# juhyeonkim95/Mitsuba3DopplerToF

Hardware: AMD Instinct MI355X
Metric: Mpaths/s (whole node), Doppler Cornell 512x512 64spp (higher is better)
Workload: dtype f32

## Files before the change

include/dtof.h:

```cpp
#ifndef DTOF_H
#define DTOF_H
#include <stdint.h>
#include <stddef.h>

#ifdef __cplusplus
extern "C" {
#endif

#define DTOF_OK            0
#define DTOF_ERR_INVALID   1
#define DTOF_ERR_HIP       2
#define DTOF_ERR_CANCELLED 3

typedef struct dtof_scene   dtof_scene;
typedef struct dtof_sampler dtof_sampler;

const char *dtof_version(void);
const char *dtof_last_error(void);

int dtof_scene_load_file(const char *path, const char *const *param_names, const char *const *param_values,
                         int n_params, dtof_scene **out);
int dtof_scene_load_string(const char *xml, const char *const *param_names, const char *const *param_values,
                           int n_params, dtof_scene **out);
void dtof_scene_destroy(dtof_scene *scene);
// ... 146 lines not shown
void dtof_sampler_destroy(dtof_sampler *s);
int  dtof_sampler_seed(dtof_sampler *s, uint32_t seed, uint32_t wavefront_size);
int  dtof_sampler_set_samples_per_wavefront(dtof_sampler *s, uint32_t spw);
int  dtof_sampler_advance(dtof_sampler *s);
int  dtof_sampler_next_1d(dtof_sampler *s, float *out);
int  dtof_sampler_next_2d(dtof_sampler *s, float *out_xy);
int  dtof_sampler_next_1d_correlate(dtof_sampler *s, const uint8_t *correlate, int correlate_all, float *out);
int  dtof_sampler_next_2d_correlate(dtof_sampler *s, const uint8_t *correlate, int correlate_all, float *out_xy);
int  dtof_sampler_next_1d_time(dtof_sampler *s, int strategy, float antithetic_shift, int stratify_each_interval, float *out);
int  dtof_sampler_get_state(dtof_sampler *s, uint32_t *out7);
int  dtof_sampler_fork(const dtof_sampler *s, dtof_sampler **out);
int  dtof_sampler_clone(const dtof_sampler *s, dtof_sampler **out);
int  dtof_sampler_set_sample_count(dtof_sampler *s, uint32_t sample_count);
int  dtof_sampler_seeded(const dtof_sampler *s);
uint32_t dtof_sampler_wavefront_size(const dtof_sampler *s);
uint32_t dtof_sampler_sample_count(const dtof_sampler *s);

int dtof_eval_modulation(dtof_scene *scene, int mode, const float *t, const float *len, float *out, uint32_t n);

int dtof_ray_intersect(dtof_scene *scene, uint32_t n, const float *rays8, float *out19, int32_t *ids3);
int dtof_ray_intersect_uv(dtof_scene *scene, uint32_t n, const float *rays8, float *out19, int32_t *ids3, float *uv4);
int dtof_ray_test(dtof_scene *scene, uint32_t n, const float *rays8, int32_t *occluded);
int dtof_flat_query(dtof_scene *scene, int form, int any, uint32_t n, const float *rays8, float *out3, int32_t *ids);

#define DTOF_COMP_MICROFACET_EVAL          0
#define DTOF_COMP_MICROFACET_PDF           1
#define DTOF_COMP_MICROFACET_G1            2
#define DTOF_COMP_MICROFACET_SAMPLE        3
#define DTOF_COMP_FRESNEL                  4
#define DTOF_COMP_FRESNEL_CONDUCTOR        5
#define DTOF_COMP_RFILTER                  6
#define DTOF_COMP_WARP_COSINE_HEMISPHERE   7
#define DTOF_COMP_WARP_DISK_CONCENTRIC     8
#define DTOF_COMP_WARP_UNIFORM_TRIANGLE    9
#define DTOF_COMP_WARP_UNIFORM_SPHERE     10
#define DTOF_COMP_COORDINATE_SYSTEM       11
#define DTOF_COMP_TEA_FLOAT32             12
#define DTOF_COMP_MATH                    13
int dtof_eval_component(int component, const float *params, int n_params, const float *in, int in_stride, float *out, int out_stride, uint32_t n);

#ifdef __cplusplus
}
#endif
#endif
```

mitsuba3dopplertof_amd/__init__.py:

```python
import ctypes as C
import os

import numpy as np

__all__ = ["load_file", "load_string", "load_dict", "Scene", "Integrator", "Sampler", "DtofError", "render",
           "render_multi_pass", "to_tof_image", "lib_path", "ETimeSampling", "velocity_map_variants", "MOMENT_PLANES", "aov_channels", "AOV_TYPES"]

_HERE = os.path.dirname(os.path.abspath(__file__))
_LIB = None


class DtofError(RuntimeError):
    pass


class ETimeSampling:
    UNIFORM, STRATIFIED, ANTITHETIC, ANTITHETIC_MIRROR, PERIODIC, REGULAR = 0, 1, 2, 3, 4, 5


class _Stats(C.Structure):
    _fields_ = [("n_paths", C.c_uint64), ("n_bounces", C.c_uint64), ("n_shadow_rays", C.c_uint64),
                ("ms_total", C.c_double), ("ms_generate", C.c_double), ("ms_trace", C.c_double),
                ("ms_shade", C.c_double), ("ms_shadow", C.c_double), ("ms_splat", C.c_double),
                ("n_launches_trace", C.c_uint32), ("n_launches_shade", C.c_uint32), ("n_launches_shadow", C.c_uint32),
# ... 96 lines not shown
    L.dtof_sampler_seeded.argtypes = [vp]
    L.dtof_eval_modulation.argtypes = [vp, C.c_int, vp, vp, vp, C.c_uint32]
    L.dtof_eval_component.argtypes = [C.c_int, vp, C.c_int, vp, C.c_int, vp, C.c_int, C.c_uint32]
    L.dtof_render_rows_async.argtypes = [vp, C.c_uint32, C.c_uint32, C.c_int32, C.c_int32, vp, C.c_int, vp]
    L.dtof_clear_async.argtypes = [vp, vp, C.c_size_t]
    L.dtof_camera_rays.argtypes = [vp, C.c_uint32, vp, vp]
    L.dtof_bsdf_eval.argtypes = [vp, C.c_uint32, C.c_uint32, vp, vp]
    L.dtof_bsdf_eval_ex.argtypes = [vp, C.c_uint32, C.c_int, C.c_uint32, vp, vp]
    L.dtof_scene_set_stream.argtypes = [vp, vp]
    L.dtof_scene_set_film_layout.argtypes = [vp, C.c_int32, C.c_uint64]
    L.dtof_render_stripes_async.argtypes = [vp, C.c_uint32, C.c_uint32, C.c_int32, C.c_int32, C.c_int32, vp, C.c_int, vp]
    L.dtof_develop_async.argtypes = [vp, vp, vp, C.c_int64]
    L.dtof_async_collect.argtypes = [vp, vp, vp, C.c_uint32, vp]
    L.dtof_ray_intersect.argtypes = [vp, C.c_uint32, vp, vp, vp]
    L.dtof_ray_intersect_uv.argtypes = [vp, C.c_uint32, vp, vp, vp, vp]
    L.dtof_ray_test.argtypes = [vp, C.c_uint32, vp, vp]
    rows, stripes = [vp, C.c_uint32, C.c_uint32, C.c_int32, C.c_int32, vp, C.c_int, vp], [vp, C.c_uint32, C.c_uint32, C.c_int32, C.c_int32, C.c_int32, vp, C.c_int, vp]
    for name, args in (("dtof_render_variants", [vp, C.c_uint32, C.c_uint32, vp, C.c_int, vp, C.POINTER(_Stats)]),
                       ("dtof_render_rows_variants", rows + [C.POINTER(_Stats)]), ("dtof_render_rows_variants_async", rows),
                       ("dtof_render_stripes_variants", stripes + [C.POINTER(_Stats)]), ("dtof_render_stripes_variants_async", stripes),
                       ("dtof_sample_lanes_variants", [vp, C.c_uint32, C.c_uint32, vp, C.c_int, C.c_uint64, C.c_uint64, vp, vp, vp]),
                       ("dtof_emitter_eval", [vp, C.c_int, C.c_int, C.c_int32, C.c_uint32, vp, vp]),
                       ("dtof_flat_query", [vp, C.c_int, C.c_int, C.c_uint32, vp, vp, vp]),
                       ("dtof_develop_accumulate_async", [vp, vp, C.c_int32, C.c_uint64, vp, C.c_int64, C.c_int]),
                       ("dtof_velocity_map_async", [vp, vp, C.c_int, vp, vp, C.c_uint32, C.c_double, C.c_double, C.c_int64, vp, vp, vp]),
                       ("dtof_velocity_map_variants", [vp, C.c_int, vp]),
                       ("dtof_render_velocity_map", [vp, C.c_uint32, C.c_uint32, vp, C.c_int, C.c_double, C.c_double, vp, vp, vp, C.POINTER(_Stats)]),
                       ("dtof_render_velocity_map_f64", [vp, C.c_uint32, C.c_uint32, vp, C.c_int, C.c_double, C.c_double, vp, vp, vp, C.POINTER(_Stats)]),
                       ("dtof_render_variants_f64", [vp, C.c_uint32, C.c_uint32, vp, C.c_int, vp, vp, C.POINTER(_Stats)]),
                       ("dtof_render_rows_variants_f64", rows[:-1] + [vp, C.c_int32, C.c_uint64, C.POINTER(_Stats)]),
                       ("dtof_develop_f64_async", [vp, vp, vp, C.c_int64]), ("dtof_develop_rgba_f64_async", [vp, vp, vp, vp, C.c_int64]),
                       ("dtof_moment_planes", [C.c_int]),
                       ("dtof_render_moments", [vp, C.c_uint32, C.c_uint32, C.c_uint32, vp, C.c_int, C.c_int, vp, C.POINTER(_Stats)]),
                       ("dtof_aov_parse", [C.c_char_p, vp, C.c_int, C.POINTER(C.c_int), vp, C.c_size_t, C.POINTER(C.c_int)]),
                       ("dtof_scene_get_aovs", [vp, vp, C.c_size_t]),
                       ("dtof_render_aovs", [vp, C.c_uint32, C.c_uint32, C.c_uint32, vp, C.c_int, C.c_int, vp, C.POINTER(_Stats)]),
                       ("dtof_sample_aov_lanes", [vp, C.c_uint32, C.c_uint32, vp, C.c_int, C.c_uint64, C.c_uint64, vp, vp])):
        if hasattr(L, name):
            getattr(L, name).argtypes = args
    _LIB = L
    return L


FLAT_GEOMETRY = np.array([[1, 0, 0,  0, 1, 0,  0, 0, 1,  1, 0, 0,  0, 1, 0,  0, 0, 1]], np.float32)


# ... 437 lines not shown

    def ray_intersect(self, o, d, time=0.0, maxt=None):
        rays = self._rays(o, d, time, maxt)
        out, ids, uv = np.zeros((len(rays), 19), np.float32), np.zeros((len(rays), 3), np.int32), np.zeros((len(rays), 4), np.float32)
        _check(_lib().dtof_ray_intersect_uv(self._h, len(rays), rays.ctypes.data, out.ctypes.data, ids.ctypes.data, uv.ctypes.data))
        return {"t": out[:, 0], "p": out[:, 1:4], "n": out[:, 4:7], "sh_n": out[:, 7:10], "sh_s": out[:, 10:13], "sh_t": out[:, 13:16],
                "wi": out[:, 16:19], "ids": ids, "uv": uv[:, 0:2], "prim_uv": uv[:, 2:4], "prim_index": ids[:, 2], "valid": ids[:, 0] >= 0}

    def ray_test(self, o, d, time=0.0, maxt=None):
        rays = self._rays(o, d, time, maxt)
        occ = np.zeros(len(rays), np.int32)
        _check(_lib().dtof_ray_test(self._h, len(rays), rays.ctypes.data, occ.ctypes.data))
        return occ != 0

    FLAT_FORMS = {"generic": 0, "one_wall": 1, "shape": 2}

    def flat_query(self, rays8, form=0, any=False):
        rays = np.ascontiguousarray(rays8, np.float32).reshape(-1, 8)
        form = self.FLAT_FORMS.get(form, form)
        out, ids = np.zeros((len(rays), 3), np.float32), np.zeros(len(rays), np.int32)
        _check(_lib().dtof_flat_query(self._h, int(form), 1 if any else 0, len(rays), rays.ctypes.data, None if any else out.ctypes.data, ids.ctypes.data))
        return ids if any else {"t": out[:, 0], "u": out[:, 1], "v": out[:, 2], "obj": ids}

    def cancel(self):
        _lib().dtof_cancel(self._h)


COMPONENTS = {"microfacet_eval": (0, 1), "microfacet_pdf": (1, 1), "microfacet_g1": (2, 1), "microfacet_sample": (3, 4), "fresnel": (4, 4),
              "fresnel_conductor": (5, 1), "rfilter": (6, 1), "warp_cosine_hemisphere": (7, 3), "warp_disk_concentric": (8, 2),
              "warp_uniform_triangle": (9, 2), "warp_uniform_sphere": (10, 3), "coordinate_system": (11, 6), "tea_float32": (12, 1), "math": (13, 1)}


def eval_component(name, inputs, params=()):
    comp, n_out = COMPONENTS[name]
    x = np.ascontiguousarray(np.atleast_2d(np.asarray(inputs, np.float32)))
    p = np.ascontiguousarray(np.asarray(params, np.float32).reshape(-1))
    out = np.zeros((len(x), n_out), np.float32)
    _check(_lib().dtof_eval_component(comp, p.ctypes.data if p.size else None, p.size, x.ctypes.data, x.shape[1], out.ctypes.data, n_out, len(x)))
    return out


class Integrator:

    def __init__(self, props):
        self.props = dict(props)
        self._h = C.c_void_p()
# ... 174 lines not shown
```

mitsuba3dopplertof_amd/csrc/dtof_flat_query.h:

```cpp
#pragma once
#include "dtof_kernels.h"

namespace dtof {

constexpr uint32_t kFlatQueryForms = 3;
constexpr uint32_t flat_query_facts(int form) { return form == 2 ? kHeadlineShapeFacts & kFactsFlatTable : form == 1 ? (uint32_t) kFactOneWall : 0u; }
void launch_flat_query(const uint8_t *scene, uint32_t scene_bytes, uint32_t flat_off, uint32_t flat_objects, uint32_t memo_obj, int form, bool any,
                       const float *rays, float *out3, int32_t *ids, uint32_t n, hipStream_t s);

}
```

mitsuba3dopplertof_amd/csrc/dtof_flat_query.hip:

```cpp
#include "dtof_device.h"
#include "dtof_flat_query.h"

namespace dtof {

static_assert(kHeadlineShapeFacts == 0 || (flat_query_facts(2) & kFactFlatShape) != 0, "form 2 is the shaped walk");

template <bool ANY, uint32_t FACTS>
__global__ __launch_bounds__(kShadeBlock) void k_flat_query(const uint8_t *scene, uint32_t scene_bytes, uint32_t stage_words, uint32_t flat_off, uint32_t flat_objects,
                                                             uint32_t memo_obj, const float *rays, float *out3, int32_t *ids, uint32_t n) {
    extern __shared__ uint4 lds[];
    constexpr bool F_ONE_WALL = (FACTS & kFactOneWall) != 0;
    const uint8_t *base = stage_scene(scene, scene_bytes, lds);
    SceneView sv = make_view(base);
    const bool have_memo = F_ONE_WALL || memo_obj != 0xffffffffu;
    sv.memo_obj = memo_obj; sv.memo = (float *) (lds + stage_words) + threadIdx.x; sv.memo_m = have_memo;
    const uint32_t i = blockIdx.x * kShadeBlock + threadIdx.x;
    if (i >= n) return;
    const float *r = rays + (size_t) i * 8;
    const V3 o = mk(r[0], r[1], r[2]), d = mk(r[3], r[4], r[5]);
    const float time = r[6], maxt = r[7];
    float memo_m[12], memo_inv[12];
    if (have_memo) instance_memo_fill(sv, time, memo_m, memo_inv);
    Hit h;
    const bool found = trace_flat<ANY, true, FACTS>(sv, (ConstBytes) scene + flat_off, flat_off, flat_objects, nullptr, o, d, time, maxt, h);
    if (ANY) { ids[i] = found ? 1 : 0; return; }
    float *w = out3 + (size_t) i * 3;
    ids[i] = found ? (int32_t) h.obj : -1;
    w[0] = found ? h.t : u2f(0x7f800000u); w[1] = found ? h.u : 0.f; w[2] = found ? h.v : 0.f;
}

template <uint32_t FACTS>
static void launch_form(bool any, uint32_t grid, uint32_t lds, hipStream_t s, const uint8_t *scene, uint32_t scene_bytes, uint32_t stage_words, uint32_t flat_off,
                        uint32_t flat_objects, uint32_t memo_obj, const float *rays, float *out3, int32_t *ids, uint32_t n) {
    if (any) hipLaunchKernelGGL((k_flat_query<true, FACTS>), dim3(grid), dim3(kShadeBlock), lds, s, scene, scene_bytes, stage_words, flat_off, flat_objects, memo_obj, rays, out3, ids, n);
    else hipLaunchKernelGGL((k_flat_query<false, FACTS>), dim3(grid), dim3(kShadeBlock), lds, s, scene, scene_bytes, stage_words, flat_off, flat_objects, memo_obj, rays, out3, ids, n);
}

void launch_flat_query(const uint8_t *scene, uint32_t scene_bytes, uint32_t flat_off, uint32_t flat_objects, uint32_t memo_obj, int form, bool any,
                       const float *rays, float *out3, int32_t *ids, uint32_t n, hipStream_t s) {
    if (!n) return;
    const uint32_t stage_words = (scene_bytes + 15u) / 16u;
    const uint32_t lds = ShadeLds::classic(stage_words, true, memo_obj != 0xffffffffu, 1u).without_stack();
    if (scene_bytes > 16u * 1024u) throw std::runtime_error("dtof_flat_query: the scene does not fit the LDS stage");
    const uint32_t grid = (n + kShadeBlock - 1u) / kShadeBlock;
    if (form == 2) launch_form<flat_query_facts(2)>(any, grid, lds, s, scene, scene_bytes, stage_words, flat_off, flat_objects, memo_obj, rays, out3, ids, n);
    else if (form == 1) launch_form<flat_query_facts(1)>(any, grid, lds, s, scene, scene_bytes, stage_words, flat_off, flat_objects, memo_obj, rays, out3, ids, n);
    else launch_form<flat_query_facts(0)>(any, grid, lds, s, scene, scene_bytes, stage_words, flat_off, flat_objects, memo_obj, rays, out3, ids, n);
}

}
```

mitsuba3dopplertof_amd/csrc/dtof_kernels.h:

```cpp
#pragma once
#include <stdint.h>
#include <hip/hip_runtime.h>
#include "dtof_math.h"

namespace dtof {

constexpr uint32_t kChunkBlocks = 8;
constexpr uint32_t kMaxInline = 4;
constexpr int kMaxOffsets = 4;

struct RenderParams {
    float s2c[16];
    float cam_to_world[12];
    float near_clip, far_clip, shutter_open, shutter_open_time;
    int32_t orthographic;
    float aperture_radius, focus_distance;
    int32_t crop_x, crop_y, crop_w, crop_h;
    float scale_x, scale_y, offset_x, offset_y;
    int32_t filter; float filter_radius, inv_radius;
    float gauss_coeff[10];
    float filter_b, filter_c;
    uint32_t base_seed, seed, seed_value;
    uint32_t spp, spp_log2;
    uint32_t tcn, pcn;
// ... 146 lines not shown
#ifndef DTOF_HEADLINE_C2
#define DTOF_HEADLINE_C2 0x3e000
#endif
constexpr uint32_t kHeadlineC2Facts = (DTOF_HEADLINE_C2) != 0 && kHeadlineFusedFacts != 0 ? (kHeadlineFusedFacts | (DTOF_HEADLINE_C2)) : 0u;
static_assert(((DTOF_HEADLINE_C2) & ~kFactsSampling) == 0, "DTOF_HEADLINE_C2 names route facts only (bits 13 and up)");
#ifndef DTOF_HEADLINE_SHAPE_COUNT
#define DTOF_HEADLINE_SHAPE_COUNT 5
#endif
#ifndef DTOF_HEADLINE_SHAPE_WALL
#define DTOF_HEADLINE_SHAPE_WALL 2
#endif
constexpr uint32_t kHeadlineShapeFacts = (DTOF_HEADLINE_SHAPE_COUNT) != 0 && (kHeadlineC2Facts & kFactOneWall) != 0 ? (kHeadlineC2Facts | flat_shape_fact(DTOF_HEADLINE_SHAPE_COUNT, DTOF_HEADLINE_SHAPE_WALL)) : 0u;
static_assert((DTOF_HEADLINE_SHAPE_COUNT) == 0 || (kHeadlineC2Facts & kFactOneWall) == 0 || (kHeadlineShapeFacts & kFactFlatShape) != 0, "a shape has 1 .. 8 objects and the wall among them");
#ifndef DTOF_HEADLINE_PAIR
#define DTOF_HEADLINE_PAIR 1
#endif
#ifndef DTOF_STREAM_JUMPS
#define DTOF_STREAM_JUMPS 1
#endif
#ifndef DTOF_PAIR_SAMPLES
#define DTOF_PAIR_SAMPLES 1
#endif
constexpr uint32_t kHeadlinePairFacts = DTOF_HEADLINE_PAIR && kHeadlineShapeFacts != 0 ? (kHeadlineShapeFacts | kFactPairSamples) : 0u;
#ifndef DTOF_FLAT_SHAPE_ANY
#define DTOF_FLAT_SHAPE_ANY 1
#endif
#ifndef DTOF_FLAT_SHAPE_CLOSEST
#define DTOF_FLAT_SHAPE_CLOSEST 1
#endif
#ifndef DTOF_WALL_FRAMES
#define DTOF_WALL_FRAMES 1
#endif
#ifndef DTOF_RESIDENT_FACTS
#define DTOF_RESIDENT_FACTS 0x37f
#endif
constexpr uint32_t kResidentFacts = DTOF_RESIDENT_FACTS;

struct ShadeLaunch { bool staged; int mode; uint32_t waves, grid, lds, lds_flat; hipStream_t stream; ShadeArgs args; uint32_t facts; };
uint32_t launch_shade_plain(bool area, bool k4, const ShadeLaunch &L);
void launch_shade_mesh(bool area, bool k4, const ShadeLaunch &L);
void launch_shade_spec1(bool k4, const ShadeLaunch &L);
void launch_shade_spec2(bool k4, const ShadeLaunch &L);
uint32_t launch_shade_resident0(bool area, bool k4, const ShadeLaunch &L);
void launch_shade_resident1(bool k4, const ShadeLaunch &L);
void launch_shade_resident2(bool k4, const ShadeLaunch &L);

// ... 70 lines not shown
```

mitsuba3dopplertof_amd/csrc/dtof_render.hip:

```cpp
#include "../../include/dtof.h"
#include "dtof_kernels.h"
#include "dtof_reconstruct.h"
#include "dtof_film64.h"
#include "dtof_moments.h"
#include "dtof_aov.h"
#include "dtof_flat_query.h"
#include "dtof_scene.h"
#include "dtof_math.h"
#include <atomic>
#include <dlfcn.h>
#include <cstdio>
#include <cstring>
#include <cstdlib>
#include <cmath>
#include <string>
#include <memory>
#include <vector>

using namespace dtof;

namespace {

thread_local std::string g_last_error;

// ... 1778 lines not shown
int dtof_flat_query(dtof_scene *sc, int form, int any, uint32_t n, const float *rays8, float *out3, int32_t *ids) {
    return guarded([&] {
        if (!sc || (n && (!rays8 || !ids || (!any && !out3)))) throw std::runtime_error("null argument");
        if (form < 0 || form >= (int) kFlatQueryForms) throw std::runtime_error("dtof_flat_query: form must be 0 (generic), 1 (one_wall) or 2 (shape)");
        if (n > (1u << 24)) throw std::runtime_error("dtof_flat_query: more than 2^24 rays in one call");
        const SceneTraits t = scene_traits(*sc);
        const FlatChoice c = flat_choice(t, t.blas_triangles <= 32768 && sc->host.textures.empty(), true, true);
        if (c.flat_objects == 0) throw std::runtime_error("dtof_flat_query: the scene has no flat table (rectangles only, at most 8 objects, fused pipeline)");
        if (form >= 1 && !(c.facts & kFactOneWall)) throw std::runtime_error("dtof_flat_query: the one_wall and shape forms need exactly one instance that holds one rectangle");
        if (form == 2 && (flat_query_facts(2) == 0 || (c.facts & kFlatShapeFields) != (flat_query_facts(2) & kFlatShapeFields)))
            throw std::runtime_error("dtof_flat_query: the shape form is compiled for a table of " + std::to_string(flat_shape_count(flat_query_facts(2))) + " rectangles with the wall at index " +
                                     std::to_string(flat_shape_wall(flat_query_facts(2))) + ", this table has " + std::to_string(c.flat_objects) + " and " + std::to_string(c.memo_obj));
        ensure_device(sc);
        DevBuf<float> dr, dout; DevBuf<int32_t> dids;
        dr.ensure((size_t) n * 8); dout.ensure(any ? 1 : (size_t) n * 3); dids.ensure(n);
        if (n) HIP_CHECK(hipMemcpy(dr.p, rays8, (size_t) n * 32, hipMemcpyHostToDevice));
        launch_flat_query(sc->d_blob.p, (uint32_t) sc->blob.size(), t.flat_off, c.flat_objects, c.memo_obj, form, any != 0, dr.p, dout.p, dids.p, n, nullptr);
        HIP_CHECK(hipGetLastError());
        if (n && !any) HIP_CHECK(hipMemcpy(out3, dout.p, (size_t) n * 12, hipMemcpyDeviceToHost));
        if (n) HIP_CHECK(hipMemcpy(ids, dids.p, (size_t) n * 4, hipMemcpyDeviceToHost));
    });
}

#ifdef DTOF_TRAVERSAL_STATS
int dtof_debug_traversal_stats_n(unsigned long long *out8, uint32_t n) {
    return guarded([&] {
        HIP_CHECK(hipDeviceSynchronize());
        unsigned long long all[kTravStats];
        if (!read_traversal_stats(all)) throw HipError("hipMemcpyFromSymbol(g_trav_stats) failed");
        for (uint32_t i = 0; i < n && i < kTravStats; ++i) out8[i] = all[i];
    });
}
int dtof_debug_traversal_stats(unsigned long long *out8) { return dtof_debug_traversal_stats_n(out8, 16); }
#endif

}
```

mitsuba3dopplertof_amd/csrc/dtof_shade.h:

```cpp
#pragma once
#include "dtof_device.h"
#include <atomic>
#include <initializer_list>
#include <type_traits>

namespace dtof {


DTOF_D uint32_t wave_append(bool pred, uint32_t &running) {
    const uint64_t mask = __ballot(pred);
    const uint32_t slot = running + (uint32_t) __popcll(mask & ((1ull << __lane_id()) - 1ull));
    running += (uint32_t) __popcll(mask);
    return slot;
}

struct BsdfOut { V3 val, weight, wo; float pdf, bs_pdf, bs_eta; bool bs_delta, bs_null; };
template <int SPEC, bool HAVE_WO = false>
DTOF_D void bsdf_eval_pdf_sample(const SceneView &sv, const DShape *sh, Surface &si, V3 wo, bool active_em, float sample_1, float s2x, float s2y, BsdfOut &out, bool want_sample = true, const V3 *diffuse_wo = nullptr) {
    const bool masked = SPEC && (sh->flags & SF_MASK);
    bool null_pick = false; float opacity = 1.f;
    if (masked) { opacity = mask_opacity_at(sv, sh, si.u, si.v); null_pick = !(sample_1 < opacity); sample_1 = sample_1 / opacity; }
    const bool blend = SPEC == 2 && (sh->flags & SF_BLEND);
    float blend_w = 0.f; bool pick_1 = false;
    if (blend) {
// ... 279 lines not shown
}
template <bool AREA, bool MESH, int SPEC, bool ONE_EMITTER = false>
void launch_emitter_eval_level(const uint8_t *scene, int mode, uint32_t index, float pmf, const float *in, float *out, uint32_t n, hipStream_t s) {
    if (n) hipLaunchKernelGGL((k_emitter_eval<AREA, MESH, SPEC, ONE_EMITTER>), dim3(nblk(n)), dim3(kBlock), 0, s, scene, mode, index, pmf, in, out, n);
}

template <bool LDS, int MODE, bool AREA, int KMAX, bool MESH, int SPEC, int RESW = 0, bool RH16 = false, uint32_t FACTS = 0>
#ifndef DTOF_MESH_WAVES
#define DTOF_MESH_WAVES 3
#endif
#ifndef DTOF_K4_RES_LDS
#define DTOF_K4_RES_LDS 1
#endif
__global__ __launch_bounds__(RESW ? RESW * 64 : kShadeBlock, RESW ? RESW / 4 : (MODE == 2 && !MESH && !SPEC && KMAX == 1) ? 4 : (MODE != 0 && MESH) ? ((SPEC && KMAX > 1) ? 2 : DTOF_MESH_WAVES) : 1) void k_shade(ShadeArgs args_by_value) {
    constexpr bool FUSED = MODE != 0, FIRST = MODE == 2;
    static_assert(FACTS == 0 || MODE == 2, "plan facts describe a first-bounce launch");
    constexpr bool F_SINGLE_PASS = (FACTS & kFactSinglePass) != 0, F_DOPPLER_CORR = (FACTS & kFactDopplerCorr) != 0, F_NO_LANE_OUT = (FACTS & kFactNoLaneOutput) != 0;
    constexpr bool F_IDENTITY = (FACTS & kFactIdentityQueue) != 0, F_NO_RR = (FACTS & kFactNoRoulette) != 0, F_CORRELATED = (FACTS & kFactCorrelated) != 0;
    constexpr bool F_WHOLE_PATH = (FACTS & kFactWholePath) != 0, F_ONE_BLOCK = (FACTS & kFactOneBlock) != 0, F_ONE_EMITTER = (FACTS & kFactOneEmitter) != 0;
    constexpr bool F_WAVE_PIXEL = (FACTS & kFactWavePixel) != 0;
    constexpr bool F_FLAT = (FACTS & kFactFlat) != 0, F_ONE_WALL = (FACTS & kFactOneWall) != 0, F_FUSED_SPLAT = (FACTS & kFactFusedSplat) != 0;
    constexpr bool F_EMITTER_SAMPLED = (FACTS & kFactEmitterSampled) != 0, F_ID24 = (FACTS & kFactIdShift24) != 0, F_SHIFTS = facts_lane_shifts(FACTS);
    constexpr bool F_PAIR = (FACTS & kFactPairSamples) != 0, JUMPS = F_PAIR && DTOF_STREAM_JUMPS, PAIR = F_PAIR && DTOF_PAIR_SAMPLES;
    static_assert(!F_PAIR || F_WAVE_PIXEL, "a lane reads its partner's registers: the whole wave is active where it does");
    static_assert(!F_PAIR || (!AREA && SPEC == 0 && KMAX == 1 && F_ONE_EMITTER), "a diffuse BSDF picks no lobe and a lone point light samples nothing: of an iteration's six draws only s2x and s2y are read");
    static_assert(!F_PAIR || (F_NO_RR && F_CORRELATED && F_DOPPLER_CORR && F_WHOLE_PATH && F_SINGLE_PASS && (FACTS & kFactStratifiedPairs) != 0), "every draw comes from the stream lanes 2k and 2k + 1 share, none is looked at for roulette, no state outlives the launch");
    constexpr bool F_FRAMES = F_ONE_WALL && DTOF_WALL_FRAMES;
    static_assert(!F_FLAT || (!MESH && SPEC == 0 && RESW == 0), "trace_flat serves the staged rectangle-only diffuse kernels");
    static_assert(!F_ONE_WALL || F_FLAT, "the one wall is an object of the flat table");
    static_assert(!F_FUSED_SPLAT || KMAX == 1, "the fused splat is the one-film kernels'");
    static_assert(!F_WAVE_PIXEL || F_IDENTITY, "whole waves of one pixel are provable for an identity queue only");
    static_assert(!F_ONE_BLOCK || RESW == 0, "blocks per segment belong to the classic launch");
    constexpr bool RES_LDS = RESW != 0 && KMAX > 1 && DTOF_K4_RES_LDS;
    constexpr bool S16 = RESW != 0 && KMAX > 1;
    static_assert(!RES_LDS || 3 * KMAX == (int) kParkWords + 1, "the film-state columns hold all but the last float of the K results");
    constexpr bool PARK_ST = DTOF_PARK && RESW == 16 && KMAX == 1;
    constexpr bool PARK = DTOF_PARK && RESW == 16 && (KMAX == 1 || RES_LDS);
    constexpr uint32_t kRngAt = RES_LDS ? kParkWords : 0u;
    constexpr int KREG = RES_LDS ? 1 : KMAX;
    constexpr uint32_t kStackStride = RESW ? RESW * 64 : kShadeBlock;
    static_assert(RESW == 0 || (MODE == 2 && !LDS && MESH), "the resident stage exists for the unstaged fused first-bounce kernel with mesh code");
    static_assert(!RH16 || RESW != 0, "half-float LDS planes belong to the resident stage");
    extern __shared__ uint4 lds[];
    __shared__ uint32_t s_inline_all[(RESW ? RESW : 1) * 2 * kMaxInline];
    typedef const char __attribute__((address_space(4))) *KernargBytes;
    const KernargBytes kernarg = (KernargBytes) __builtin_amdgcn_kernarg_segment_ptr();
// ... 157 lines not shown
                pair_wo_next = mk(__int_as_float(__builtin_amdgcn_update_dpp(0, __float_as_int(mine.x), 0xf5, 0xf, 0xf, false)),
                                  __int_as_float(__builtin_amdgcn_update_dpp(0, __float_as_int(mine.y), 0xf5, 0xf, 0xf, false)),
                                  __int_as_float(__builtin_amdgcn_update_dpp(0, __float_as_int(mine.z), 0xf5, 0xf, 0xf, false)));
            }
            if (PARK) park_store();
            pos_reg = pl.pos;
            if (!fuse_splat) {
                q.pos[l] = pl.pos;
                q.rng_b[l] = make_uint2((uint32_t) (main.inc >> 1), (uint32_t) (path.inc >> 1));
            }
            if (dbg) {
                LaneDebug &o = dbg[l];
                o.time = ra.w; o.ray_o[0] = ra.x; o.ray_o[1] = ra.y; o.ray_o[2] = ra.z; o.ray_d[0] = rb.x; o.ray_d[1] = rb.y; o.ray_d[2] = rb.z;
            }
            if (have_memo) instance_memo_fill(sv, ra.w, memo_m, memo_inv);
            if constexpr (F_FRAMES) {
                const DShape &ws = sv.shapes[sv.groups[sv.objects[sv.memo_obj].index].first_shape];
                wf.n = normalize(xf_normal(memo_inv, mk(ws.n[0], ws.n[1], ws.n[2])));
                const V3 du = xf_vector(memo_m, mk(ws.dp_du[0], ws.dp_du[1], ws.dp_du[2]));
                wf.s = normalize(vfma(wf.n, -dot(wf.n, du), du));
                if (du.x == 0.f && du.y == 0.f && du.z == 0.f) { V3 tt; coordinate_system(wf.n, wf.s, tt); }
            }
            Hit h;
            bool found = (F_FLAT || flat) ? trace_flat<false, true, FACTS & kFactsFlatTable>(sv, (ConstBytes) A.scene + rp.flat_off, rp.flat_off, flat, stack, mk(ra.x, ra.y, ra.z), mk(rb.x, rb.y, rb.z), ra.w, rb.w, h)
                              : trace_scene<false, MESH, FUSED, RESW != 0, kStackStride, S16, 0u, false, RH16>(sv, stack, mk(ra.x, ra.y, ra.z), mk(rb.x, rb.y, rb.z), ra.w, rb.w, h);
            hh = make_uint4(f2u(h.t), f2u(h.u), f2u(h.v), h.prim);
            hid = found ? (h.obj | (h.shape << (F_ID24 ? 24u : q.id_shift))) : 0xffffffffu;
        }
    }
    const uint32_t n_inline = FIRST ? rp.inline_iters : 1u;
    for (uint32_t it = 0; ; ++it) {
    const uint32_t depth = depth0 + it;
    const bool last = it + 1 >= n_inline;
    const uint32_t trace_next = last ? trace_next_last : 1u;
    const bool terminal = last && (F_WHOLE_PATH || rp.terminal != 0);
    alive = false; want_shadow = false;
    if (lane_on) {
        if (PARK) park_load();
        if (!FIRST) {
            hid = q.hit_id[l];
            if (hid != 0xffffffffu) {
                ra = q.ray_a[l]; rb = q.ray_b[l]; hh = load_hit<MESH>(q, l); st = q.st_a[l];
                const uint4 rs = q.rng_a[l]; const uint2 ri = q.rng_b[l];
                main.state = (uint64_t) rs.x | ((uint64_t) rs.y << 32); main.inc = ((uint64_t) ri.x << 1) | 1u;
                path.state = (uint64_t) rs.z | ((uint64_t) rs.w << 32); path.inc = ((uint64_t) ri.y << 1) | 1u;
            }
        }
// ... 354 lines not shown
```

mitsuba3dopplertof_amd/csrc/dtof_traverse.h:

```cpp
#pragma once
#include "dtof_kernels.h"
#include "dtof_scene.h"
#include "dtof_math.h"
#include "dtof_flat_cull.h"

#ifndef DTOF_D
#define DTOF_D __device__ __forceinline__
#endif

namespace dtof {

struct SceneView {
    const DNode *nodes; const DNode16 *nodes16; const DObject *objects; const DGroup *groups; const DShape *shapes;
    const DTri *tris; const DTriIsect *isect; const DTriShade *shading; const DEmitter *emitters; const uint8_t *base;
    uint32_t n_nodes, n_emitters;
    uint32_t memo_obj; float *memo;
    bool memo_m;
};
constexpr uint32_t kResNodes = 1024;
constexpr uint32_t kLeafFlag16 = 0x8000u, kNoChild16 = 0xffffu, kDone16 = 0x7fffu;
DTOF_D uint32_t encode_child16(uint32_t w) { return w == kNoChild ? kNoChild16 : ((w & 0x7fffu) | ((w >> 16) & 0x8000u)); }
DTOF_D SceneView make_view(const uint8_t *base) {
    const BlobHeader *h = (const BlobHeader *) base;
    SceneView v;
    v.nodes = (const DNode *) (base + h->off_nodes);
    v.nodes16 = (const DNode16 *) (base + h->off_nodes16);
    v.objects = (const DObject *) (base + h->off_objects);
// ... 354 lines not shown
    bool r = false;
    if (active) r = trace_scene<ANY, MESH, MEMO, SOA, STRIDE, false, LDSN, TL, H16, DEFER>(sv, stack, o, d, time, maxt, best, ovf, tlas, cand);
    return r;
}
template <bool ANY, int MESH, uint32_t STRIDE, uint32_t LDSN, bool H16>
DTOF_D bool trace_deferred(const SceneView &sv, uint32_t *stack, uint4 cand, V3 o, V3 d, float time, float maxt, Hit &best, uint32_t *ovf) {
    const uint32_t stride = STRIDE ? STRIDE : blockDim.x;
    const uint32_t c[4] = { cand.x, cand.y, cand.z, cand.w };
#pragma unroll 1
    for (int i = 0; i < 4; ++i) {
        if (c[i] == 0xffffffffu) break;
        if (intersect_object<ANY, MESH, false, STRIDE, false, LDSN, H16>(sv, c[i], o, d, time, maxt, best, stack, 0, stride, ovf) && ANY) return true;
    }
    return best.obj != 0xffffffffu;
}


typedef const uint8_t __attribute__((address_space(4))) *ConstBytes;
typedef float F2 __attribute__((ext_vector_type(2)));
struct FlatRecord { F2 c0, c1, c2, c3; };
DTOF_D F2 flat_zrow(float z0, float z1, float z2, float z3, V3 ro, V3 rd) {
    return F2{ fmaf(z2, ro.z, fmaf(z1, ro.y, fmaf(z0, ro.x, z3))), fmaf(z2, rd.z, fmaf(z1, rd.y, z0 * rd.x)) };
}
template <bool ANY, bool MEMO, uint32_t FACTS = 0>
DTOF_D bool trace_flat(const SceneView &sv, ConstBytes flat_table, uint32_t flat_off, uint32_t n_objects, uint32_t *stack, V3 o, V3 d, float time, float maxt, Hit &best) {
    best.t = maxt; best.u = best.v = 0.f; best.obj = 0xffffffffu; best.shape = 0; best.prim = 0;
    bool occluded = false;
    DTOF_STAT(0);
    auto test = [&](const FlatRecord &rec, uint32_t oi, V3 ro, V3 rd, F2 z) {
        const F2 lo_xy = F2{ fmaf(rec.c2.x, ro.z, fmaf(rec.c1.x, ro.y, fmaf(rec.c0.x, ro.x, rec.c3.x))), fmaf(rec.c2.y, ro.z, fmaf(rec.c1.y, ro.y, fmaf(rec.c0.y, ro.x, rec.c3.y))) };
        const F2 ld_xy = F2{ fmaf(rec.c2.x, rd.z, fmaf(rec.c1.x, rd.y, rec.c0.x * rd.x)), fmaf(rec.c2.y, rd.z, fmaf(rec.c1.y, rd.y, rec.c0.y * rd.x)) };
        const float t = -z.x / z.y;
        const float u = fmaf(ld_xy.x, t, lo_xy.x), v = fmaf(ld_xy.y, t, lo_xy.y);
        const bool hit = (int) (t >= 0.f) & (int) (t <= maxt) & (int) (fabsf(u) <= 1.f) & (int) (fabsf(v) <= 1.f);
        if (ANY) occluded |= hit;
        else {
            const bool take = (int) hit & (int) (t < best.t);
            best.t = take ? t : best.t; best.u = take ? u : best.u; best.v = take ? v : best.v; best.obj = take ? oi : best.obj;
        }
    };
    constexpr bool F_ONE_WALL = (FACTS & kFactOneWall) != 0;
    static_assert(!F_ONE_WALL || MEMO, "the one wall is the memo object");
    const DFlatObject *lt = (const DFlatObject *) (sv.base + flat_off);
    const uint4 *zt = (const uint4 *) (lt + n_objects) + 1;
    constexpr int kStat = ANY ? 16 : 20; (void) kStat;
    const float far = flat_cull_far(maxt);
    uint32_t oi = 0;
    if constexpr (F_ONE_WALL) {
        auto visit = [&](uint32_t k, const V3 &ro, const V3 &rd) {
            const uint4 zr = zt[k];
            const F2 z = flat_zrow(u2f(zr.x), u2f(zr.y), u2f(zr.z), u2f(zr.w), ro, rd);
            const bool need = !flat_certain_miss(z.x, z.y, far);
            DTOF_STAT(kStat); DTOF_STAT_WAVE(kStat + 2);
            if (!need) DTOF_STAT(kStat + 1);
            if (!__ballot(need)) return;
            DTOF_STAT_WAVE(kStat + 3);
            const uint4 *rp4 = (const uint4 *) (lt + k);
            const uint4 r0 = rp4[0], r1 = rp4[1], r2 = rp4[2], r3 = rp4[3];
            FlatRecord a;
            a.c0 = F2{ u2f(r0.x), u2f(r0.y) }; a.c1 = F2{ u2f(r1.x), u2f(r1.y) }; a.c2 = F2{ u2f(r2.x), u2f(r2.y) }; a.c3 = F2{ u2f(r3.x), u2f(r3.y) };
            test(a, k, ro, rd, z);
        };
        constexpr uint32_t N = flat_shape_count(FACTS), WALL = flat_shape_wall(FACTS);
        if constexpr (N != 0 && ANY && DTOF_FLAT_SHAPE_ANY) {
            const DFlatObject *lts = (const DFlatObject *) (sv.base + flat_off);
            const uint4 *zts = (const uint4 *) (lts + N) + 1;
            float inv[12]; instance_memo_load(sv, inv);
            const V3 wo = xf_point(inv, o), wd = xf_vector(inv, d);
            bool any_need = false;
#pragma unroll
            for (uint32_t k = 0; k < N; ++k) {
                const uint4 zr = zts[k];
                const F2 z = k == WALL ? flat_zrow(u2f(zr.x), u2f(zr.y), u2f(zr.z), u2f(zr.w), wo, wd) : flat_zrow(u2f(zr.x), u2f(zr.y), u2f(zr.z), u2f(zr.w), o, d);
                const bool need = !flat_certain_miss(z.x, z.y, far);
                DTOF_STAT(kStat); DTOF_STAT_WAVE(kStat + 2);
                if (!need) DTOF_STAT(kStat + 1);
                any_need |= need;
                if ((k & 1u) != 0) __builtin_amdgcn_sched_barrier(0);
            }
            if (!__ballot(any_need)) return false;
#pragma unroll 1
            for (uint32_t k = 0; k < N; ++k) {
                const bool is_wall = k == WALL;
                const V3 ro = is_wall ? wo : o, rd = is_wall ? wd : d;
                const uint4 zr = zts[k];
                const F2 z = flat_zrow(u2f(zr.x), u2f(zr.y), u2f(zr.z), u2f(zr.w), ro, rd);
// ... 4 lines not shown
                const uint4 r0 = rp4[0], r1 = rp4[1], r2 = rp4[2], r3 = rp4[3];
                FlatRecord a;
                a.c0 = F2{ u2f(r0.x), u2f(r0.y) }; a.c1 = F2{ u2f(r1.x), u2f(r1.y) }; a.c2 = F2{ u2f(r2.x), u2f(r2.y) }; a.c3 = F2{ u2f(r3.x), u2f(r3.y) };
                test(a, k, ro, rd, z);
            }
            return occluded;
        } else if constexpr (N != 0 && !ANY && DTOF_FLAT_SHAPE_CLOSEST) {
            const DFlatObject *lts = (const DFlatObject *) (sv.base + flat_off);
            const uint4 *zts = (const uint4 *) (lts + N) + 1;
            auto visit_at = [&](uint32_t k, const V3 &ro, const V3 &rd) {
                const uint4 zr = zts[k];
                const F2 z = flat_zrow(u2f(zr.x), u2f(zr.y), u2f(zr.z), u2f(zr.w), ro, rd);
                const bool need = !flat_certain_miss(z.x, z.y, far);
                DTOF_STAT(kStat); DTOF_STAT_WAVE(kStat + 2);
                if (!need) DTOF_STAT(kStat + 1);
                if (!__ballot(need)) return;
                DTOF_STAT_WAVE(kStat + 3);
                const uint4 *rp4 = (const uint4 *) (lts + k);
                const uint4 r0 = rp4[0], r1 = rp4[1], r2 = rp4[2], r3 = rp4[3];
                FlatRecord a;
                a.c0 = F2{ u2f(r0.x), u2f(r0.y) }; a.c1 = F2{ u2f(r1.x), u2f(r1.y) }; a.c2 = F2{ u2f(r2.x), u2f(r2.y) }; a.c3 = F2{ u2f(r3.x), u2f(r3.y) };
                test(a, k, ro, rd, z);
            };
#pragma unroll
            for (uint32_t k = 0; k < N; ++k) {
                if (k == WALL) {
                    float inv[12]; instance_memo_load(sv, inv);
                    const V3 wo = xf_point(inv, o), wd = xf_vector(inv, d);
                    visit_at(k, wo, wd);
                } else visit_at(k, o, d);
                __builtin_amdgcn_sched_barrier(0);
            }
            return best.obj != 0xffffffffu;
        }
        const uint32_t wall = sv.memo_obj;
#pragma unroll 1
        for (uint32_t seg = 0; seg < 2u; ++seg) {
            const uint32_t end = seg ? n_objects : wall;
            for (; oi < end; ++oi) visit(oi, o, d);
            if (seg == 0) {
                float inv[12]; instance_memo_load(sv, inv);
                const V3 wo = xf_point(inv, o), wd = xf_vector(inv, d);
                visit(oi++, wo, wd);
            }
        }
    } else {
// ... 35 lines not shown
```

Baseline: 19020.

## Split flat-table primary-ray walk across lane pairs sharing the same ray

```diff
diff --git a/include/dtof.h b/include/dtof.h
--- a/include/dtof.h
+++ b/include/dtof.h
@@ -192,6 +192,7 @@
 int dtof_ray_intersect_uv(dtof_scene *scene, uint32_t n, const float *rays8, float *out19, int32_t *ids3, float *uv4);
 int dtof_ray_test(dtof_scene *scene, uint32_t n, const float *rays8, int32_t *occluded);
 int dtof_flat_query(dtof_scene *scene, int form, int any, uint32_t n, const float *rays8, float *out3, int32_t *ids);
+int dtof_flat_query_pairs(dtof_scene *scene, int any, uint32_t n, const float *rays8, float *out3, int32_t *ids);
 
 #define DTOF_COMP_MICROFACET_EVAL          0
 #define DTOF_COMP_MICROFACET_PDF           1
diff --git a/mitsuba3dopplertof_amd/__init__.py b/mitsuba3dopplertof_amd/__init__.py
--- a/mitsuba3dopplertof_amd/__init__.py
+++ b/mitsuba3dopplertof_amd/__init__.py
@@ -142,6 +142,7 @@
                        ("dtof_sample_lanes_variants", [vp, C.c_uint32, C.c_uint32, vp, C.c_int, C.c_uint64, C.c_uint64, vp, vp, vp]),
                        ("dtof_emitter_eval", [vp, C.c_int, C.c_int, C.c_int32, C.c_uint32, vp, vp]),
                        ("dtof_flat_query", [vp, C.c_int, C.c_int, C.c_uint32, vp, vp, vp]),
+                       ("dtof_flat_query_pairs", [vp, C.c_int, C.c_uint32, vp, vp, vp]),
                        ("dtof_develop_accumulate_async", [vp, vp, C.c_int32, C.c_uint64, vp, C.c_int64, C.c_int]),
                        ("dtof_velocity_map_async", [vp, vp, C.c_int, vp, vp, C.c_uint32, C.c_double, C.c_double, C.c_int64, vp, vp, vp]),
                        ("dtof_velocity_map_variants", [vp, C.c_int, vp]),
@@ -625,6 +626,12 @@
         _check(_lib().dtof_flat_query(self._h, int(form), 1 if any else 0, len(rays), rays.ctypes.data, None if any else out.ctypes.data, ids.ctypes.data))
         return ids if any else {"t": out[:, 0], "u": out[:, 1], "v": out[:, 2], "obj": ids}
 
+    def flat_query_pairs(self, rays8, any=False):
+        rays = np.ascontiguousarray(rays8, np.float32).reshape(-1, 8)
+        out, ids = np.zeros((len(rays), 3), np.float32), np.zeros(len(rays), np.int32)
+        _check(_lib().dtof_flat_query_pairs(self._h, 1 if any else 0, len(rays), rays.ctypes.data, None if any else out.ctypes.data, ids.ctypes.data))
+        return ids if any else {"t": out[:, 0], "u": out[:, 1], "v": out[:, 2], "obj": ids}
+
     def cancel(self):
         _lib().dtof_cancel(self._h)
 
diff --git a/mitsuba3dopplertof_amd/csrc/dtof_flat_query.h b/mitsuba3dopplertof_amd/csrc/dtof_flat_query.h
--- a/mitsuba3dopplertof_amd/csrc/dtof_flat_query.h
+++ b/mitsuba3dopplertof_amd/csrc/dtof_flat_query.h
@@ -5,6 +5,8 @@
 
 constexpr uint32_t kFlatQueryForms = 3;
 constexpr uint32_t flat_query_facts(int form) { return form == 2 ? kHeadlineShapeFacts & kFactsFlatTable : form == 1 ? (uint32_t) kFactOneWall : 0u; }
+constexpr int kFlatQueryPairs = 3;
+constexpr bool kFlatQueryPairsBuilt = pair_walk_shape(flat_query_facts(2));
 void launch_flat_query(const uint8_t *scene, uint32_t scene_bytes, uint32_t flat_off, uint32_t flat_objects, uint32_t memo_obj, int form, bool any,
                        const float *rays, float *out3, int32_t *ids, uint32_t n, hipStream_t s);
 
diff --git a/mitsuba3dopplertof_amd/csrc/dtof_flat_query.hip b/mitsuba3dopplertof_amd/csrc/dtof_flat_query.hip
--- a/mitsuba3dopplertof_amd/csrc/dtof_flat_query.hip
+++ b/mitsuba3dopplertof_amd/csrc/dtof_flat_query.hip
@@ -5,9 +5,9 @@
 
 static_assert(kHeadlineShapeFacts == 0 || (flat_query_facts(2) & kFactFlatShape) != 0, "form 2 is the shaped walk");
 
-template <bool ANY, uint32_t FACTS>
-__global__ __launch_bounds__(kShadeBlock) void k_flat_query(const uint8_t *scene, uint32_t scene_bytes, uint32_t stage_words, uint32_t flat_off, uint32_t flat_objects,
-                                                             uint32_t memo_obj, const float *rays, float *out3, int32_t *ids, uint32_t n) {
+template <bool ANY, uint32_t FACTS, bool PAIR_RAYS>
+DTOF_D void flat_query_lane(const uint8_t *scene, uint32_t scene_bytes, uint32_t stage_words, uint32_t flat_off, uint32_t flat_objects,
+                            uint32_t memo_obj, const float *rays, float *out3, int32_t *ids, uint32_t n) {
     extern __shared__ uint4 lds[];
     constexpr bool F_ONE_WALL = (FACTS & kFactOneWall) != 0;
     const uint8_t *base = stage_scene(scene, scene_bytes, lds);
@@ -22,11 +22,21 @@
     float memo_m[12], memo_inv[12];
     if (have_memo) instance_memo_fill(sv, time, memo_m, memo_inv);
     Hit h;
-    const bool found = trace_flat<ANY, true, FACTS>(sv, (ConstBytes) scene + flat_off, flat_off, flat_objects, nullptr, o, d, time, maxt, h);
+    const bool found = trace_flat<ANY, true, FACTS, PAIR_RAYS>(sv, (ConstBytes) scene + flat_off, flat_off, flat_objects, nullptr, o, d, time, maxt, h);
     if (ANY) { ids[i] = found ? 1 : 0; return; }
     float *w = out3 + (size_t) i * 3;
     ids[i] = found ? (int32_t) h.obj : -1;
     w[0] = found ? h.t : u2f(0x7f800000u); w[1] = found ? h.u : 0.f; w[2] = found ? h.v : 0.f;
+}
+template <bool ANY, uint32_t FACTS>
+__global__ __launch_bounds__(kShadeBlock) void k_flat_query(const uint8_t *scene, uint32_t scene_bytes, uint32_t stage_words, uint32_t flat_off, uint32_t flat_objects,
+                                                             uint32_t memo_obj, const float *rays, float *out3, int32_t *ids, uint32_t n) {
+    flat_query_lane<ANY, FACTS, false>(scene, scene_bytes, stage_words, flat_off, flat_objects, memo_obj, rays, out3, ids, n);
+}
+template <bool ANY>
+__global__ __launch_bounds__(kShadeBlock) void k_flat_query_pairs(const uint8_t *scene, uint32_t scene_bytes, uint32_t stage_words, uint32_t flat_off, uint32_t flat_objects,
+                                                                   uint32_t memo_obj, const float *rays, float *out3, int32_t *ids, uint32_t n) {
+    if constexpr (kFlatQueryPairsBuilt) flat_query_lane<ANY, flat_query_facts(2), true>(scene, scene_bytes, stage_words, flat_off, flat_objects, memo_obj, rays, out3, ids, n);
 }
 
 template <uint32_t FACTS>
@@ -43,7 +53,10 @@
     const uint32_t lds = ShadeLds::classic(stage_words, true, memo_obj != 0xffffffffu, 1u).without_stack();
     if (scene_bytes > 16u * 1024u) throw std::runtime_error("dtof_flat_query: the scene does not fit the LDS stage");
     const uint32_t grid = (n + kShadeBlock - 1u) / kShadeBlock;
-    if (form == 2) launch_form<flat_query_facts(2)>(any, grid, lds, s, scene, scene_bytes, stage_words, flat_off, flat_objects, memo_obj, rays, out3, ids, n);
+    if (form == kFlatQueryPairs) {
+        if (any) hipLaunchKernelGGL((k_flat_query_pairs<true>), dim3(grid), dim3(kShadeBlock), lds, s, scene, scene_bytes, stage_words, flat_off, flat_objects, memo_obj, rays, out3, ids, n);
+        else hipLaunchKernelGGL((k_flat_query_pairs<false>), dim3(grid), dim3(kShadeBlock), lds, s, scene, scene_bytes, stage_words, flat_off, flat_objects, memo_obj, rays, out3, ids, n);
+    } else if (form == 2) launch_form<flat_query_facts(2)>(any, grid, lds, s, scene, scene_bytes, stage_words, flat_off, flat_objects, memo_obj, rays, out3, ids, n);
     else if (form == 1) launch_form<flat_query_facts(1)>(any, grid, lds, s, scene, scene_bytes, stage_words, flat_off, flat_objects, memo_obj, rays, out3, ids, n);
     else launch_form<flat_query_facts(0)>(any, grid, lds, s, scene, scene_bytes, stage_words, flat_off, flat_objects, memo_obj, rays, out3, ids, n);
 }
diff --git a/mitsuba3dopplertof_amd/csrc/dtof_kernels.h b/mitsuba3dopplertof_amd/csrc/dtof_kernels.h
--- a/mitsuba3dopplertof_amd/csrc/dtof_kernels.h
+++ b/mitsuba3dopplertof_amd/csrc/dtof_kernels.h
@@ -192,6 +192,15 @@
 #define DTOF_PAIR_SAMPLES 1
 #endif
 constexpr uint32_t kHeadlinePairFacts = DTOF_HEADLINE_PAIR && kHeadlineShapeFacts != 0 ? (kHeadlineShapeFacts | kFactPairSamples) : 0u;
+#ifndef DTOF_PAIR_WALK_PRIMARY
+#define DTOF_PAIR_WALK_PRIMARY 1
+#endif
+#ifdef DTOF_TRAVERSAL_STATS
+constexpr bool kPairWalkCompiled = false;
+#else
+constexpr bool kPairWalkCompiled = true;
+#endif
+constexpr bool pair_walk_shape(uint32_t facts) { return (facts & kFactOneWall) != 0 && flat_shape_count(facts) == 5 && flat_shape_wall(facts) == 2; }
 #ifndef DTOF_FLAT_SHAPE_ANY
 #define DTOF_FLAT_SHAPE_ANY 1
 #endif
diff --git a/mitsuba3dopplertof_amd/csrc/dtof_pair_walk.h b/mitsuba3dopplertof_amd/csrc/dtof_pair_walk.h
--- /dev/null
+++ b/mitsuba3dopplertof_amd/csrc/dtof_pair_walk.h
@@ -0,0 +1,25 @@
+#pragma once
+#include <stdint.h>
+
+#ifndef DTOF_HD
+#if defined(__HIP__)
+#define DTOF_HD __host__ __device__ __forceinline__
+#else
+#define DTOF_HD inline
+#endif
+#endif
+
+namespace dtof {
+
+struct FlatBest { float t, u, v; uint32_t obj; };
+
+DTOF_HD void flat_best_take(FlatBest &b, bool hit, float t, float u, float v, uint32_t oi) {
+    const bool take = (int) hit & (int) (t < b.t);
+    b.t = take ? t : b.t; b.u = take ? u : b.u; b.v = take ? v : b.v; b.obj = take ? oi : b.obj;
+}
+DTOF_HD void pair_merge_upper(FlatBest &b, const FlatBest &upper) {
+    const bool take = upper.t < b.t;
+    b.t = take ? upper.t : b.t; b.u = take ? upper.u : b.u; b.v = take ? upper.v : b.v; b.obj = take ? upper.obj : b.obj;
+}
+
+}
diff --git a/mitsuba3dopplertof_amd/csrc/dtof_render.hip b/mitsuba3dopplertof_amd/csrc/dtof_render.hip
--- a/mitsuba3dopplertof_amd/csrc/dtof_render.hip
+++ b/mitsuba3dopplertof_amd/csrc/dtof_render.hip
@@ -1824,6 +1824,32 @@
     });
 }
 
+int dtof_flat_query_pairs(dtof_scene *sc, int any, uint32_t n, const float *rays8, float *out3, int32_t *ids) {
+    return guarded([&] {
+        if (!sc || (n && (!rays8 || !ids || (!any && !out3)))) throw std::runtime_error("null argument");
+        if (n & 1u) throw std::runtime_error("dtof_flat_query_pairs: an odd number of rays");
+        if (n > (1u << 24)) throw std::runtime_error("dtof_flat_query_pairs: more than 2^24 rays in one call");
+        for (uint32_t i = 0; i < n; i += 2) {
+            const float *a = rays8 + (size_t) i * 8, *b = a + 8;
+            if (memcmp(a, b, 24) != 0 || memcmp(a + 7, b + 7, 4) != 0)
+                throw std::runtime_error("dtof_flat_query_pairs: rays " + std::to_string(i) + " and " + std::to_string(i + 1) + " differ in o, d or maxt");
+        }
+        const SceneTraits t = scene_traits(*sc);
+        const FlatChoice c = flat_choice(t, t.blas_triangles <= 32768 && sc->host.textures.empty(), true, true);
+        if (!kFlatQueryPairsBuilt || c.flat_objects == 0 || !(c.facts & kFactOneWall) || (c.facts & kFlatShapeFields) != (flat_query_facts(2) & kFlatShapeFields))
+            throw std::runtime_error("dtof_flat_query_pairs: the pair form is compiled for a flat table of 5 rectangles whose one instance, of one rectangle, is at index 2" +
+                                     (c.flat_objects ? ", this table has " + std::to_string(c.flat_objects) + " objects" : std::string(", this scene has no flat table")));
+        ensure_device(sc);
+        DevBuf<float> dr, dout; DevBuf<int32_t> dids;
+        dr.ensure((size_t) n * 8); dout.ensure(any ? 1 : (size_t) n * 3); dids.ensure(n);
+        if (n) HIP_CHECK(hipMemcpy(dr.p, rays8, (size_t) n * 32, hipMemcpyHostToDevice));
+        launch_flat_query(sc->d_blob.p, (uint32_t) sc->blob.size(), t.flat_off, c.flat_objects, c.memo_obj, kFlatQueryPairs, any != 0, dr.p, dout.p, dids.p, n, nullptr);
+        HIP_CHECK(hipGetLastError());
+        if (n && !any) HIP_CHECK(hipMemcpy(out3, dout.p, (size_t) n * 12, hipMemcpyDeviceToHost));
+        if (n) HIP_CHECK(hipMemcpy(ids, dids.p, (size_t) n * 4, hipMemcpyDeviceToHost));
+    });
+}
+
 #ifdef DTOF_TRAVERSAL_STATS
 int dtof_debug_traversal_stats_n(unsigned long long *out8, uint32_t n) {
     return guarded([&] {
diff --git a/mitsuba3dopplertof_amd/csrc/dtof_shade.h b/mitsuba3dopplertof_amd/csrc/dtof_shade.h
--- a/mitsuba3dopplertof_amd/csrc/dtof_shade.h
+++ b/mitsuba3dopplertof_amd/csrc/dtof_shade.h
@@ -325,6 +325,7 @@
     constexpr bool F_FLAT = (FACTS & kFactFlat) != 0, F_ONE_WALL = (FACTS & kFactOneWall) != 0, F_FUSED_SPLAT = (FACTS & kFactFusedSplat) != 0;
     constexpr bool F_EMITTER_SAMPLED = (FACTS & kFactEmitterSampled) != 0, F_ID24 = (FACTS & kFactIdShift24) != 0, F_SHIFTS = facts_lane_shifts(FACTS);
     constexpr bool F_PAIR = (FACTS & kFactPairSamples) != 0, JUMPS = F_PAIR && DTOF_STREAM_JUMPS, PAIR = F_PAIR && DTOF_PAIR_SAMPLES;
+    constexpr bool WALK_PRIMARY = F_PAIR && DTOF_PAIR_WALK_PRIMARY && pair_walk_shape(FACTS);
     static_assert(!F_PAIR || F_WAVE_PIXEL, "a lane reads its partner's registers: the whole wave is active where it does");
     static_assert(!F_PAIR || (!AREA && SPEC == 0 && KMAX == 1 && F_ONE_EMITTER), "a diffuse BSDF picks no lobe and a lone point light samples nothing: of an iteration's six draws only s2x and s2y are read");
     static_assert(!F_PAIR || (F_NO_RR && F_CORRELATED && F_DOPPLER_CORR && F_WHOLE_PATH && F_SINGLE_PASS && (FACTS & kFactStratifiedPairs) != 0), "every draw comes from the stream lanes 2k and 2k + 1 share, none is looked at for roulette, no state outlives the launch");
@@ -528,7 +529,7 @@
                 if (du.x == 0.f && du.y == 0.f && du.z == 0.f) { V3 tt; coordinate_system(wf.n, wf.s, tt); }
             }
             Hit h;
-            bool found = (F_FLAT || flat) ? trace_flat<false, true, FACTS & kFactsFlatTable>(sv, (ConstBytes) A.scene + rp.flat_off, rp.flat_off, flat, stack, mk(ra.x, ra.y, ra.z), mk(rb.x, rb.y, rb.z), ra.w, rb.w, h)
+            bool found = (F_FLAT || flat) ? trace_flat<false, true, FACTS & kFactsFlatTable, WALK_PRIMARY>(sv, (ConstBytes) A.scene + rp.flat_off, rp.flat_off, flat, stack, mk(ra.x, ra.y, ra.z), mk(rb.x, rb.y, rb.z), ra.w, rb.w, h)
                               : trace_scene<false, MESH, FUSED, RESW != 0, kStackStride, S16, 0u, false, RH16>(sv, stack, mk(ra.x, ra.y, ra.z), mk(rb.x, rb.y, rb.z), ra.w, rb.w, h);
             hh = make_uint4(f2u(h.t), f2u(h.u), f2u(h.v), h.prim);
             hid = found ? (h.obj | (h.shape << (F_ID24 ? 24u : q.id_shift))) : 0xffffffffu;
diff --git a/mitsuba3dopplertof_amd/csrc/dtof_traverse.h b/mitsuba3dopplertof_amd/csrc/dtof_traverse.h
--- a/mitsuba3dopplertof_amd/csrc/dtof_traverse.h
+++ b/mitsuba3dopplertof_amd/csrc/dtof_traverse.h
@@ -3,6 +3,7 @@
 #include "dtof_scene.h"
 #include "dtof_math.h"
 #include "dtof_flat_cull.h"
+#include "dtof_pair_walk.h"
 
 #ifndef DTOF_D
 #define DTOF_D __device__ __forceinline__
@@ -403,7 +404,7 @@
 DTOF_D F2 flat_zrow(float z0, float z1, float z2, float z3, V3 ro, V3 rd) {
     return F2{ fmaf(z2, ro.z, fmaf(z1, ro.y, fmaf(z0, ro.x, z3))), fmaf(z2, rd.z, fmaf(z1, rd.y, z0 * rd.x)) };
 }
-template <bool ANY, bool MEMO, uint32_t FACTS = 0>
+template <bool ANY, bool MEMO, uint32_t FACTS = 0, bool PAIR_RAYS = false>
 DTOF_D bool trace_flat(const SceneView &sv, ConstBytes flat_table, uint32_t flat_off, uint32_t n_objects, uint32_t *stack, V3 o, V3 d, float time, float maxt, Hit &best) {
     best.t = maxt; best.u = best.v = 0.f; best.obj = 0xffffffffu; best.shape = 0; best.prim = 0;
     bool occluded = false;
@@ -443,6 +444,8 @@
             test(a, k, ro, rd, z);
         };
         constexpr uint32_t N = flat_shape_count(FACTS), WALL = flat_shape_wall(FACTS);
+        constexpr bool PAIR = PAIR_RAYS && kPairWalkCompiled;
+        static_assert(!PAIR_RAYS || pair_walk_shape(FACTS), "the pair form is written for five rectangles with the wall at index 2: {0, 1} below it, {3, 4} above");
         if constexpr (N != 0 && ANY && DTOF_FLAT_SHAPE_ANY) {
             const DFlatObject *lts = (const DFlatObject *) (sv.base + flat_off);
             const uint4 *zts = (const uint4 *) (lts + N) + 1;
@@ -493,6 +496,44 @@
                 a.c0 = F2{ u2f(r0.x), u2f(r0.y) }; a.c1 = F2{ u2f(r1.x), u2f(r1.y) }; a.c2 = F2{ u2f(r2.x), u2f(r2.y) }; a.c3 = F2{ u2f(r3.x), u2f(r3.y) };
                 test(a, k, ro, rd, z);
             };
+            if constexpr (PAIR) {
+                const uint32_t first = (__lane_id() & 1u) * (WALL + 1u);
+                const DFlatObject *ltp = lts + first;
+                const uint4 *ztp = zts + first;
+#pragma unroll
+                for (uint32_t s = 0; s < 2u; ++s) {
+                    const uint4 zr = ztp[s];
+                    const F2 z = flat_zrow(u2f(zr.x), u2f(zr.y), u2f(zr.z), u2f(zr.w), o, d);
+                    const bool need = !flat_certain_miss(z.x, z.y, far);
+                    if (__ballot(need)) {
+                        const uint4 *rp4 = (const uint4 *) (ltp + s);
+                        const uint4 r0 = rp4[0], r1 = rp4[1], r2 = rp4[2], r3 = rp4[3];
+                        FlatRecord a;
+                        a.c0 = F2{ u2f(r0.x), u2f(r0.y) }; a.c1 = F2{ u2f(r1.x), u2f(r1.y) }; a.c2 = F2{ u2f(r2.x), u2f(r2.y) }; a.c3 = F2{ u2f(r3.x), u2f(r3.y) };
+                        test(a, first + s, o, d, z);
+                    }
+                    __builtin_amdgcn_sched_barrier(0);
+                }
+                FlatBest upper;
+                upper.t = __int_as_float(__builtin_amdgcn_update_dpp(0, __float_as_int(best.t), 0xf5, 0xf, 0xf, false));
+                upper.u = __int_as_float(__builtin_amdgcn_update_dpp(0, __float_as_int(best.u), 0xf5, 0xf, 0xf, false));
+                upper.v = __int_as_float(__builtin_amdgcn_update_dpp(0, __float_as_int(best.v), 0xf5, 0xf, 0xf, false));
+                upper.obj = (uint32_t) __builtin_amdgcn_update_dpp(0, (int) best.obj, 0xf5, 0xf, 0xf, false);
+                best.t = __int_as_float(__builtin_amdgcn_update_dpp(0, __float_as_int(best.t), 0xa0, 0xf, 0xf, false));
+                best.u = __int_as_float(__builtin_amdgcn_update_dpp(0, __float_as_int(best.u), 0xa0, 0xf, 0xf, false));
+                best.v = __int_as_float(__builtin_amdgcn_update_dpp(0, __float_as_int(best.v), 0xa0, 0xf, 0xf, false));
+                best.obj = (uint32_t) __builtin_amdgcn_update_dpp(0, (int) best.obj, 0xa0, 0xf, 0xf, false);
+                {
+                    float inv[12]; instance_memo_load(sv, inv);
+                    const V3 wo = xf_point(inv, o), wd = xf_vector(inv, d);
+                    visit_at(WALL, wo, wd);
+                }
+                __builtin_amdgcn_sched_barrier(0);
+                FlatBest b{ best.t, best.u, best.v, best.obj };
+                pair_merge_upper(b, upper);
+                best.t = b.t; best.u = b.u; best.v = b.v; best.obj = b.obj;
+                return best.obj != 0xffffffffu;
+            }
 #pragma unroll
             for (uint32_t k = 0; k < N; ++k) {
                 if (k == WALL) {
```

Result: faster. 19270, median of 6 (+1.3%).
